# Rickyeeeeee/ParallelRayTracing

Hardware: AMD Instinct MI355X
Metric: Mrays/sec at 1920x1080, 4 bounces, ~1M-tri scene (higher is better)
Workload: dtype f32; 1 GPU; C3: dragon.ply refined by longest-edge bisection = 870000 triangles + ground quad + emissive quad, 1920x1080, max_depth 5 segments (= 4 bounces), 256 spp per step (15360 spp timed of the config's 256), image tiled over 1 GPU(s) + per-step gather to rank 0; triangles=870000, bvh_nodes=681504, bvh_max_depth=25, bvh8_nodes=137301, bvh8_depth=9, width=1920, height=1080, max_depth=5, samples_in_flight=256, seed=0, jitter=0, variant=0, gather=render stream

## Files before the change

include/prt.h:

```cpp
#ifndef PRT_H
#define PRT_H

#include <stddef.h>
#include <stdint.h>

#ifdef __cplusplus
extern "C" {
#endif

#define PRT_VERSION 1

enum {
    PRT_OK = 0,
    PRT_ERR_INVALID = 1,
    PRT_ERR_NO_DEVICE = 2,
    PRT_ERR_HIP = 3,
    PRT_ERR_IO = 4,
    PRT_ERR_NOMEM = 5
};

enum { PRT_SHAPE_CIRCLE = 0, PRT_SHAPE_QUAD = 1, PRT_SHAPE_TRIANGLE = 2 };
enum { PRT_MAT_NONE = 0, PRT_MAT_LAMBERTIAN = 1, PRT_MAT_METAL = 2, PRT_MAT_DIELECTRIC = 3, PRT_MAT_EMISSIVE = 4 };
enum {
    PRT_PRESET_DEFAULT = 0, PRT_PRESET_LIGHT_TEST = 1, PRT_PRESET_MATERIAL_TEST = 2, PRT_PRESET_CORNELL = 3,
// ... 450 lines not shown

int prt_enable_timing(PrtContext* ctx, int on);
int prt_get_stats(PrtContext* ctx, PrtStats* out);
int prt_reset_stats(PrtContext* ctx);
int prt_measure_traversal(PrtContext* ctx, uint32_t max_depth, uint32_t seed, uint32_t sample, PrtStats* out);
int prt_measure_shade_divergence(PrtContext* ctx, uint32_t max_depth, uint32_t seed, uint32_t sample, uint64_t* out);
int prt_bvh_info(PrtContext* ctx, PrtBvhInfo* out);
uint32_t prt_spill_rows(uint32_t max_stack4, uint32_t max_depth);
int prt_kernel_occupancy(PrtContext* ctx, PrtOccupancy* out);
int prt_kernel_instance(PrtContext* ctx, char* name, uint32_t capacity);
int prt_shade_instance(PrtContext* ctx, char* name, uint32_t capacity);
enum { PRT_STAGE_RAYGEN = 0, PRT_STAGE_SHADE0 = 1, PRT_STAGE_SHADE = 2, PRT_STAGE_ACCUMULATE = 3 };
int prt_batch_instance(PrtContext* ctx, uint32_t stage, char* name, uint32_t capacity);
int prt_instance_name(uint32_t stage, uint32_t index, char* name, uint32_t capacity);
int prt_last_segment(PrtContext* ctx, uint32_t* active, uint32_t* front_rays);
int prt_primary_reuse(PrtContext* ctx, uint32_t* active, uint32_t* reused_batches);
int prt_bvh_read(PrtContext* ctx, float* nodes, float* tris);
int prt_bvh_read4(PrtContext* ctx, float* nodes4);
int prt_bvh_read8(PrtContext* ctx, uint32_t* nodes8);
int prt_set_variant(PrtContext* ctx, int variant);
int prt_set_param(PrtContext* ctx, const char* name, int value);

typedef struct PrtGroup PrtGroup;
int prt_group_create(const int* device_ids, uint32_t n, PrtGroup** out);
void prt_group_destroy(PrtGroup* g);
const char* prt_group_last_error(const PrtGroup* g);
uint32_t prt_group_size(const PrtGroup* g);
const char* prt_group_transport(const PrtGroup* g);
PrtContext* prt_group_context(PrtGroup* g, uint32_t rank);
int prt_group_set_scene(PrtGroup* g, const PrtSceneDesc* scene);
// ... 59 lines not shown
```

parallelraytracing_amd/capi.py:

```python
from __future__ import annotations

import ctypes as C
import os

_HERE = os.path.dirname(os.path.abspath(__file__))
LIB_PATH = os.environ.get("PRT_LIB_PATH") or os.path.join(_HERE, "csrc", "libprt.so")

PRT_MAX_DEPTH = 64

SHAPE_CIRCLE, SHAPE_QUAD, SHAPE_TRIANGLE = 0, 1, 2
MAT_NONE, MAT_LAMBERTIAN, MAT_METAL, MAT_DIELECTRIC, MAT_EMISSIVE = 0, 1, 2, 3, 4
(PRESET_DEFAULT, PRESET_LIGHT_TEST, PRESET_MATERIAL_TEST, PRESET_CORNELL, PRESET_RANDOM_BALLS_SMALL,
 PRESET_RANDOM_BALLS_MEDIUM, PRESET_RANDOM_BALLS_LARGE) = range(7)
PRESET_NAMES = {
    "DEFAULT": PRESET_DEFAULT, "LIGHT_TEST": PRESET_LIGHT_TEST, "MATERIAL_TEST": PRESET_MATERIAL_TEST,
    "CORNELL": PRESET_CORNELL, "RANDOM_BALLS_SMALL": PRESET_RANDOM_BALLS_SMALL,
    "RANDOM_BALLS_MEDIUM": PRESET_RANDOM_BALLS_MEDIUM, "RANDOM_BALLS_LARGE": PRESET_RANDOM_BALLS_LARGE,
}


class PrtMaterial(C.Structure):
    _fields_ = [("type", C.c_uint32), ("rgb", C.c_float * 3), ("scalar", C.c_float)]


# ... 356 lines not shown
                                                 _vp, _vp, C.POINTER(PrtBakeInfo)]),
    "prt_bake_light_samples": (C.c_int, [_vp, C.POINTER(PrtBakeTarget), C.c_uint32, C.c_uint32, _fp, _fp, _u32p, _fp, _fp]),
    "prt_enable_timing": (C.c_int, [_vp, C.c_int]),
    "prt_get_stats": (C.c_int, [_vp, C.POINTER(PrtStats)]),
    "prt_reset_stats": (C.c_int, [_vp]),
    "prt_measure_traversal": (C.c_int, [_vp, C.c_uint32, C.c_uint32, C.c_uint32, C.POINTER(PrtStats)]),
    "prt_bvh_info": (C.c_int, [_vp, C.POINTER(PrtBvhInfo)]),
    "prt_spill_rows": (C.c_uint32, [C.c_uint32, C.c_uint32]),
    "prt_kernel_occupancy": (C.c_int, [_vp, C.POINTER(PrtOccupancy)]),
    "prt_kernel_instance": (C.c_int, [_vp, C.c_char_p, C.c_uint32]),
    "prt_shade_instance": (C.c_int, [_vp, C.c_char_p, C.c_uint32]),
    "prt_batch_instance": (C.c_int, [_vp, C.c_uint32, C.c_char_p, C.c_uint32]),
    "prt_instance_name": (C.c_int, [C.c_uint32, C.c_uint32, C.c_char_p, C.c_uint32]),
    "prt_last_segment": (C.c_int, [_vp, C.POINTER(C.c_uint32), C.POINTER(C.c_uint32)]),
    "prt_primary_reuse": (C.c_int, [_vp, C.POINTER(C.c_uint32), C.POINTER(C.c_uint32)]),
    "prt_measure_shade_divergence": (C.c_int, [_vp, C.c_uint32, C.c_uint32, C.c_uint32, C.POINTER(C.c_uint64)]),
    "prt_refit_meshes": (C.c_int, [_vp, C.POINTER(PrtMesh), C.c_uint32]),
    "prt_refit_meshes_device": (C.c_int, [_vp, C.POINTER(PrtMeshDeviceArrays), C.c_uint32]),
    "prt_mesh_normals_device": (C.c_int, [_vp, C.c_uint32, _vp, _vp]),
    "prt_refit_info": (C.c_int, [_vp, C.POINTER(PrtRefitInfo)]),
    "prt_set_instance_transforms": (C.c_int, [_vp, C.POINTER(PrtInstance), C.c_uint32, C.c_uint32]),
    "prt_group_set_instance_transforms": (C.c_int, [_vp, C.POINTER(PrtInstance), C.c_uint32, C.c_uint32]),
    "prt_instance_update_info": (C.c_int, [_vp, C.POINTER(PrtInstanceUpdateInfo)]),
    "prt_instances_read": (C.c_int, [_vp, C.c_uint32, _u32p, _u32p, _u32p, _u32p, _u32p]),
    "prt_bvh_read": (C.c_int, [_vp, _fp, _fp]),
    "prt_set_sampling": (C.c_int, [_vp, C.POINTER(PrtSampling)]),
    "prt_bvh_read4": (C.c_int, [_vp, _fp]),
    "prt_bvh_read8": (C.c_int, [_vp, C.POINTER(C.c_uint32)]),
    "prt_set_variant": (C.c_int, [_vp, C.c_int]),
    "prt_set_param": (C.c_int, [_vp, C.c_char_p, C.c_int]),
# ... 46 lines not shown
```

parallelraytracing_amd/csrc/prt_api.cpp:

```cpp
#include <hip/hip_runtime.h>

#include <algorithm>
#include <cfloat>
#include <chrono>
#include <cmath>
#include <cstdarg>
#include <cstdio>
#include <cstdlib>
#include <cstring>
#include <limits>
#include <string>
#include <utility>
#include <vector>

#include "../../include/prt.h"
#include "bvh.h"
#include "bvh_gpu.h"
#include "prt_adaptive.h"
#include "prt_denoise.h"
#include "prt_denoise_contract.h"
#include "prt_feature_samples.h"
#include "prt_features.h"
#include "prt_kernels.h"
#include "prt_primary_cache.h"
// ... 100 lines not shown
    int measure_spp = 1;
    float pad_coeff = kPadCoeff;
    int node_stride = 0;
    int compact_primary = 1;
    int primary_walk = 1;
    const char* shade_instance = "";
    const char* batch_instance[4] = {"", "", "", ""};
    bool batch_walked = false;
    int gpu_build = 0;
    PrtSampling sampling{0u, 0u, 0.0f};
    PrtLens lens{0.0f, 0.0f, 0.0f};
    PrtTravTuning tune{1024u, 256u, 16u, 0xFFFFFFFFu , 0u, 2u, 0u , 0u, 0u, 0u, 1u, 8u, 1u, 0u, nullptr, 0u, 2500000u, 2u , 8u , 96u , 32u , 1u};
    unsigned long long* d_shade_div = nullptr;
    uint32_t last_segment = 2;
    uint32_t last_segment_active = 0;
    uint32_t last_batch_depth = 0;
    uint32_t sort_rays = 0;
    uint32_t* d_sort = nullptr;
    size_t sort_entries = 0, sort_temp = 0;
    uint32_t* h_counts = nullptr;
    hipEvent_t ev_counts[PRT_MAX_DEPTH + 2] = {};
    hipEvent_t ev_prod[PRT_MAX_DEPTH + 2] = {};
    hipStream_t count_stream = nullptr;
    uint32_t* d_work = nullptr;
    float4* d_pix = nullptr;
    uint32_t pix_entries = 0;
    uint32_t* d_prim_pid = nullptr;
    uint32_t* d_prim_list = nullptr;
    uint32_t* d_prim_hit = nullptr;
    uint64_t prim_pid_entries = 0;
// ... 676 lines not shown
    EventPair ep{};
    auto accumulate_batch = [&]() -> int {
        if ((rc = begin_event(c, 3, &ep))) return rc;
        const PrtAccumulateArgs aa{c->d_rad, lit ? c->lb.lrad : nullptr, c->d_film_local, c->d_film_stat, tm, S_cur, max_depth,
                                   accumulate, c->ray_stats_target, compact ? c->d_pix + tm.n_pix_local : nullptr, view.list};
        if (!prt_launch_accumulate(c->stream, plan.accumulate, aa)) return fail(c, PRT_ERR_INVALID, "no such accumulate instance");
        c->batch_instance[PRT_STAGE_ACCUMULATE] = prt_accumulate_name(plan.accumulate);
        if ((rc = end_event(c, &ep))) return rc;
        if (accumulate && !view.list) c->stats.samples += S_cur;
        HIPCHECK(c, hipGetLastError());
        return PRT_OK;
    };
    c->shade_instance = "";
    for (const char*& n : c->batch_instance) n = "";
    c->last_segment_active = plan.last_segment;
    c->last_batch_depth = plan.path ? 0u : max_depth;
    if (plan.path) {
        HIPCHECK(c, hipMemsetAsync(c->d_work, 0, 256 * sizeof(uint32_t), c->stream));
        PrtPathArgs pa{c->cam, tm, c->sampling, c->d_rad, first_sample, seed, max_depth, n_paths};
        if ((rc = begin_event(c, 1, &ep))) return rc;
        prt_launch_path(c->stream, prt_plan_walk(wf), c->dsc, pa, c->d_work, c->tune);
        if ((rc = end_event(c, &ep))) return rc;
        ++c->stats.intersect_launches;
        return accumulate_batch();
    }
    if (compact && c->pix_entries < tm.n_pix_local) {
        free_dev(c->d_pix);
        c->pix_entries = 0;
        c->primary_key.valid = false;
        HIPCHECK(c, hipMalloc((void**)&c->d_pix, 4 * (size_t)tm.n_pix_local * sizeof(float4)));
// ... 79 lines not shown
            }
        }
        uint32_t n_rays_known = 0xFFFFFFFFu;
        if (exact && held) {
            n_rays_known = c->primary_counts[0] + c->primary_counts[1];
        } else if (exact) {
            HIPCHECK(c, hipEventSynchronize(c->ev_counts[d]));
            n_rays_known = c->h_counts[64 * (size_t)d] + c->h_counts[64 * (size_t)d + 32];
            if (d == 0) c->primary_counts[0] = c->h_counts[0], c->primary_counts[1] = c->h_counts[32];
        }
        if (n_rays_known == 0u) break;
        if (d == 0 && !reuse && now.valid) c->primary_key = now;
        if (c->d_shade_div) prt_launch_shade_divstats(c->stream, c->dsc, in, c->d_counts, d, n_paths, c->d_shade_div, prim_d);
        if ((rc = begin_event(c, 2, &ep))) return rc;
        const PrtShadeInst shade = d == 0 ? plan.shade0 : plan.shade;
        const PrtShadeArgs sa{&c->dsc, in, out, c->d_rad, c->d_counts, c->d_work, d, max_depth, n_paths, c->sampling, n_rays_known, prim_d, plan.last_segment,
                              f.env ? &denv : nullptr, f.tex ? &dtex : nullptr, lit ? &lt : nullptr, (lit && f.mesh_lights) ? &mlt : nullptr,
                              lit ? &c->lb : nullptr, (lit && f.light_clusters) ? &lct : nullptr};
        if (!prt_launch_shade(c->stream, shade, sa)) return fail(c, PRT_ERR_INVALID, "no such shade instance");
        c->shade_instance = prt_shade_name(shade);
        c->batch_instance[(d == 0 && plan.shade0 != plan.shade) ? PRT_STAGE_SHADE0 : PRT_STAGE_SHADE] = c->shade_instance;
        if (lit && (lt.n_lights || (f.env && (denv.t_all | denv.t_env)))) {
            const uint32_t* scount = c->d_counts + (size_t)d * PRT_CNT_STRIDE + 48u;
            const uint32_t nmax = n_rays_known == 0xFFFFFFFFu ? n_paths : n_rays_known;
            prt_launch_scan_prims_bounded(c->stream, c->dsc, c->lb.sh, scount, c->d_work, nmax);
            if (c->dsc.n_nodes) walk_rays(c, c->lb.sh, scount, nmax, true, c->tune, nullptr, nullptr);
            prt_launch_light_accum(c->stream, c->dsc, c->lb, scount, c->d_work, nmax);
        }
        if ((rc = end_event(c, &ep))) return rc;
        if (exact && d + 1 < max_depth) HIPCHECK(c, read_back(d + 1));
    }
    return accumulate_batch();
}
// ... 3058 lines not shown
int prt_last_segment(PrtContext* c, uint32_t* active, uint32_t* front_rays) {
    if (!c || !active) return PRT_ERR_INVALID;
    *active = c->last_segment_active;
    if (front_rays) {
        *front_rays = 0u;
        if (c->last_batch_depth != 0u && c->d_counts) {
            HIPCHECK(c, hipSetDevice(c->device));
            HIPCHECK(c, hipStreamSynchronize(c->stream));
            HIPCHECK(c, hipMemcpy(front_rays, c->d_counts + (size_t)(c->last_batch_depth - 1u) * PRT_CNT_STRIDE, sizeof(uint32_t),
                                  hipMemcpyDeviceToHost));
        }
    }
    return PRT_OK;
}

int prt_primary_reuse(PrtContext* c, uint32_t* active, uint32_t* reused_batches) {
    if (!c || !active) return PRT_ERR_INVALID;
    *active = c->primary_reuse_active;
    if (reused_batches) *reused_batches = c->primary_reused_batches;
    return PRT_OK;
}

int prt_bvh_info(PrtContext* c, PrtBvhInfo* out) {
    if (!c || !out) return PRT_ERR_INVALID;
    if (!c->has_scene) return fail(c, PRT_ERR_INVALID, "prt_set_scene has not been called");
    *out = c->hs.bvh_info;
    return PRT_OK;
}

int prt_bvh_read4(PrtContext* c, float* nodes4) {
// ... 27 lines not shown
    const std::string n = name;
    if (n == "variant") c->variant = value;
    else if (n == "primary_reuse" && (value == 0 || value == 1)) c->primary_reuse = value;
    else if (n == "grid_blocks" && value > 0 && value <= 8192) c->tune.grid_blocks = (uint32_t)value;
    else if (n == "chunk" && value >= 64 && value % 64 == 0) c->tune.chunk = (uint32_t)value;
    else if (n == "xcd_affinity" && (value == 0 || value == 1)) c->tune.xcd_affinity = (uint32_t)value;
    else if (n == "wide" && (value == 0 || value == 1 || value == 2)) c->tune.wide = (uint32_t)value;
    else if (n == "stack_lds" && (value == 0 || value == 1 || value == 2 || value == 3 || value == 4 || value == 5 || value == 6 || value == 24 || value == 39)) c->tune.stack_lds = (uint32_t)value;
    else if (n == "exact_grids" && (value == 0 || value == 1 || value == 2)) c->tune.exact_grids = (uint32_t)value;
    else if (n == "steal" && value >= 0 && value <= 64) c->tune.steal = (uint32_t)value;
    else if (n == "primary_hit" && (value == 0 || value == 1)) c->tune.primary_hit = (uint32_t)value;
    else if (n == "path_kernel" && value >= 0 && value <= 2) c->tune.path_kernel = (uint32_t)value;
    else if (n == "path_max" && value >= 1) c->tune.path_max = (uint32_t)value;
    else if (n == "sort_rays" && value >= 0 && value <= 2) c->sort_rays = (uint32_t)value;
    else if (n == "last_segment" && value >= 0 && value <= 2) c->last_segment = (uint32_t)value;
    else if (n == "compact_primary" && (value == 0 || value == 1)) c->compact_primary = value;
    else if (n == "primary_walk" && (value == 0 || value == 1)) c->primary_walk = value;
    else if (n == "node_stride" && (value == 0 || value == 5 || value == 8)) c->node_stride = value;
    else if (n == "pad_log2" && value >= 8 && value <= 22) c->pad_coeff = std::ldexp(1.0f, -value);
    else if (n == "tail" && value >= 0 && value <= 64) c->tune.tail = (uint32_t)value;
    else if (n == "big" && value >= 1 && value <= 16) c->tune.big = (uint32_t)value;
    else if (n == "static_small" && value >= 0 && value <= 4096) c->tune.static_small = (uint32_t)value;
    else if (n == "big_min" && value >= 1 && value <= 100000) c->tune.big_min = (uint32_t)value;
    else if (n == "big_keep" && value >= 0 && value <= 1024) c->tune.big_keep = (uint32_t)value;
    else if (n == "stack_cap" && value >= 0 && value <= 64) c->tune.stack_cap = (uint32_t)value;
    else if (n == "prim_bvh" && (value == 0 || value == 1)) c->abvh_enabled = value;
    else if (n == "measure_spp" && value >= 1 && value <= 1024) c->measure_spp = value;
    else if (n == "gpu_build" && (value == 0 || value == 1 || value == 2)) c->gpu_build = value;
    else if (n == "fuse" && (value == 0 || value == 1)) c->tune.fuse = (uint32_t)value;
    else if (n == "tri_min" && value >= 0 && value <= 1024) c->tune.tri_min = (uint32_t)value;
// ... 20 lines not shown
```

parallelraytracing_amd/csrc/prt_kernels.h:

```cpp
#pragma once
#include <hip/hip_runtime_api.h>
#include <hip/hip_vector_types.h>
#include <stdint.h>

#include "../../include/prt.h"
#include "prt_route.h"
#include "prt_walk.h"
#include "prt_scene_pod.h"

struct f3 {
    float x, y, z;
};

struct DevCamera {
    f3 pos, front, right, up;
    float W, H, tan_fov_y;
};
struct DevLens {
    float aperture, focus;
};

#define PRT_DIR_MIN 9.094947017729282e-13f

struct DevScene {
// ... 140 lines not shown
                           uint32_t* work, uint32_t max_rays, unsigned long long* stats);
struct PrtWalkArgs {
    const DevScene* sc;
    PrtRayBuf rays;
    const uint32_t* count;
    uint32_t* work;
    uint32_t* spill;
    unsigned long long* stats;
    const PrtPrimary* primary;
    const PrtTravTuning* tune;
};
void prt_launch_walk(hipStream_t st, const PrtWalkPlan& plan, const PrtWalkArgs& a);
void prt_launch_path(hipStream_t st, const PrtWalkPlan& plan, const DevScene& sc, const PrtPathArgs& pa, uint32_t* work, const PrtTravTuning& tune);
int prt_walk_occupancy(const PrtWalkPlan& plan, int* blocks_per_cu, int* vgprs, int* sgprs, int* lds_bytes);
#define PRT_LAST_SEGMENT_FLAG 0x80000000u
struct PrtShadeArgs {
    const DevScene* sc;
    PrtRayBuf in, out;
    float4* rad;
    uint32_t* counts;
    uint32_t* work;
    uint32_t depth, max_depth, cap;
    PrtSampling sp;
    uint32_t n_rays_known;
    const PrtPrimary* primary;
    uint32_t last_segment;
    const DevEnv* env;
    const DevTex* tex;
    const DevLights* lights;
    const DevMeshLights* mesh_lights;
    const PrtLightBufs* lb;
    const DevLightClusters* clusters;
};
bool prt_launch_shade(hipStream_t st, PrtShadeInst inst, const PrtShadeArgs& a);
void prt_launch_shade_divstats(hipStream_t st, const DevScene& sc, const PrtRayBuf& in, const uint32_t* counts, uint32_t iter,
                               uint32_t cap, unsigned long long* out, const PrtPrimary* primary = nullptr);
void prt_launch_primary_hit(hipStream_t st, const DevScene& sc, const PrtPrimary& pr, const uint32_t* hit, float4* pix,
                            const uint32_t* counts);
struct PrtAccumulateArgs {
    const float4* rad;
    const float4* lrad;
    float4* film_local;
    float2* stat;
    PrtTileMap tm;
    uint32_t S, max_depth;
    bool update_film;
    unsigned long long* ray_stats;
    const float4* pix_end;
    const uint32_t* list;
// ... 36 lines not shown
```

parallelraytracing_amd/csrc/prt_kernels.hip:

```cpp
#include "prt_kernels.h"

#include "prt_adaptive.h"
#include "prt_device.h"

#define HIT_MISS 0xFFFFFFFFu
#define HIT_DEAD 0xFFFFFFFEu

PRT_DEV uint32_t xcd_remap(uint32_t b, uint32_t n) {
    const uint32_t q = n >> 3, r = n & 7u;
    const uint32_t xcd = b & 7u, i = b >> 3;
    const uint32_t start = xcd < r ? xcd * (q + 1u) : r * (q + 1u) + (xcd - r) * q;
    return start + i;
}

#define CNT_STRIDE PRT_CNT_STRIDE
#define CNT_A(c, d) (c)[(d) * CNT_STRIDE]
#define CNT_B(c, d) (c)[(d) * CNT_STRIDE + 32u]
#define CNT_C(c, d) (c)[(d) * CNT_STRIDE + 16u]
#define PRODUCER_BLOCK 1024
#ifndef SHADE_BLOCK
#define SHADE_BLOCK 512
#endif

template <int BLOCK>
PRT_DEV uint32_t block_alloc2(bool front, bool back, bool done, uint32_t* cntA, uint32_t* cntB, uint32_t* cntC,
                              uint32_t cap, uint32_t mult = 1u, uint32_t* stride = nullptr, uint32_t* base = nullptr) {
    __shared__ uint32_t s_a[BLOCK / 64], s_b[BLOCK / 64], s_c[BLOCK / 64];
    __shared__ uint32_t s_base_a, s_base_b, s_tot_a, s_tot_b;
    const unsigned long long ma = __ballot(front), mb = __ballot(back), mc = __ballot(done);
    const uint32_t lane = lane_id(), wave = threadIdx.x >> 6;
    if (lane == 0) {
        s_a[wave] = (uint32_t)__popcll(ma);
        s_b[wave] = (uint32_t)__popcll(mb);
        s_c[wave] = (uint32_t)__popcll(mc);
    }
    __syncthreads();
    if (threadIdx.x == 0) {
        uint32_t ta = 0, tb = 0, tc = 0;
        for (uint32_t w = 0; w < BLOCK / 64; ++w) {
            ta += s_a[w];
            tb += s_b[w];
            tc += s_c[w];
        }
// ... 2121 lines not shown
    traverse8_body<STACK_L, WAVES, false, INST, LEAN, false, false, true>(sc, ro, rd, hit, hd2, count_ptr, work, ovf, tune,
                                                                          nullptr, PrtPrimary{}, PrtPathArgs{});
}

template <int STACK_L, int WAVES, bool INST, bool LEAN = false>
__global__ void __launch_bounds__(256, WAVES) k_occluded8_seeded(DevScene sc, const float4* __restrict__ ro,
                                                                const float4* __restrict__ rd, uint32_t* __restrict__ hit,
                                                                const float* __restrict__ hd2,
                                                                const uint32_t* __restrict__ count_ptr,
                                                                uint32_t* __restrict__ work, uint32_t* __restrict__ ovf,
                                                                PrtTravTuning tune) {
    traverse8_body<STACK_L, WAVES, false, INST, LEAN, false, false, true, true>(sc, ro, rd, hit, hd2, count_ptr, work, ovf, tune,
                                                                                nullptr, PrtPrimary{}, PrtPathArgs{});
}

template <int FUSE, bool SAMPLING, bool INST, bool ABVH, bool PRIM, bool ENV, bool TEX = false>
PRT_DEV void shade_step(DevScene sc, const float4* __restrict__ ro, const float4* __restrict__ rd, const float4* __restrict__ rt,
                        const uint32_t* __restrict__ hit, float4* __restrict__ no, float4* __restrict__ nd, float4* __restrict__ nt,
                        uint32_t* __restrict__ nhit, float* __restrict__ nhd2, float4* __restrict__ rad, uint32_t* __restrict__ counts,
                        uint32_t* __restrict__ work, uint32_t iter, uint32_t max_depth_arg, uint32_t cap, PrtSampling sp_arg, PrtPrimary pr,
                        const DevEnv* env, const DevTex* tex = nullptr) {
    const bool last_route = (max_depth_arg & PRT_LAST_SEGMENT_FLAG) != 0u;
    const uint32_t max_depth = max_depth_arg & ~PRT_LAST_SEGMENT_FLAG;
    const PrtSampling sp = SAMPLING ? sp_arg : PrtSampling{0u, 0u, 0.0f};
    const uint32_t nA = CNT_A(counts, iter), nB = CNT_B(counts, iter);
    const uint32_t count = nA + nB;
    if (blockIdx.x * (uint32_t)SHADE_BLOCK >= count) return;
    const uint32_t k = blockIdx.x * (uint32_t)SHADE_BLOCK + threadIdx.x;
    if (k < 8u) work[32u * k] = 0u;
    if (k == 8u) work[512] = 0u;
    bool front = false, back = false;
    f3 o = mk3(0.f, 0.f, 0.f), d = mk3(0.f, 0.f, 1.f), thr = mk3(0.f, 0.f, 0.f);
    uint32_t id0 = HIT_MISS, rng = 0, depth = 0, pid = 0;
    float d2_0 = 3.402823466e+38f;
    float4 pre_a = make_float4(0.f, 0.f, 0.f, 0.f), pre_b = pre_a;
    if (k < count) {
        const uint32_t src = k < nA ? k : cap - 1u - (k - nA);
        uint32_t id = (PRIM && (k >= nA || pr.walk)) ? HIT_MISS : ld_stream(&hit[src]);
        if (PRIM) {
            pid = ld_stream(&pr.pid[src]);
            uint32_t pixel, sample, lp;
            primary_ray(pr, pid, o, d, pixel, sample, &lp);
            if (k >= nA) id = __float_as_uint(pr.pix[pr.n_pix_local + lp].y);
            else if (pr.walk) id = hit[__float_as_uint(pr.pix[pr.n_pix_local + lp].x)];
            rng = path_seed(pixel, pr.first_sample + sample, pr.seed);
// ... 29 lines not shown
    }
}

template <int FUSE, bool SAMPLING, bool INST, bool ABVH, bool PRIM = false>
__global__ void __launch_bounds__(SHADE_BLOCK) k_shade(DevScene sc, const float4* __restrict__ ro,
                                                      const float4* __restrict__ rd, const float4* __restrict__ rt,
                                                      const uint32_t* __restrict__ hit, float4* __restrict__ no,
                                                      float4* __restrict__ nd, float4* __restrict__ nt,
                                                      uint32_t* __restrict__ nhit, float* __restrict__ nhd2,
                                                      float4* __restrict__ rad, uint32_t* __restrict__ counts,
                                                      uint32_t* __restrict__ work, uint32_t iter, uint32_t max_depth,
                                                      uint32_t cap, PrtSampling sp_arg, PrtPrimary pr) {
    shade_step<FUSE, SAMPLING, INST, ABVH, PRIM, false>(sc, ro, rd, rt, hit, no, nd, nt, nhit, nhd2, rad, counts, work, iter, max_depth,
                                                        cap, sp_arg, pr, nullptr);
}

template <bool INST, bool ABVH>
__global__ void __launch_bounds__(SHADE_BLOCK) k_shade_env(DevScene sc, DevEnv env, const float4* __restrict__ ro,
                                                          const float4* __restrict__ rd, const float4* __restrict__ rt,
                                                          const uint32_t* __restrict__ hit, float4* __restrict__ no,
                                                          float4* __restrict__ nd, float4* __restrict__ nt,
                                                          uint32_t* __restrict__ nhit, float* __restrict__ nhd2,
                                                          float4* __restrict__ rad, uint32_t* __restrict__ counts,
                                                          uint32_t* __restrict__ work, uint32_t iter, uint32_t max_depth,
                                                          uint32_t cap, PrtSampling sp_arg) {
    shade_step<0, true, INST, ABVH, false, true>(sc, ro, rd, rt, hit, no, nd, nt, nhit, nhd2, rad, counts, work, iter, max_depth, cap,
                                                 sp_arg, PrtPrimary{}, &env);
}

template <bool INST, bool ABVH, bool ENV>
// ... 29 lines not shown
            }
        }
    }
    pix[2u * pr.n_pix_local + pl] = a;
    pix[3u * pr.n_pix_local + pl] = b;
}

__global__ void __launch_bounds__(SHADE_BLOCK) k_shade_divstats(DevScene sc, const uint32_t* __restrict__ hit,
                                                                 const uint32_t* __restrict__ counts, uint32_t iter, uint32_t cap,
                                                                 unsigned long long* __restrict__ out, PrtPrimary pr, int compact) {
    const uint32_t nA = CNT_A(counts, iter), nB = CNT_B(counts, iter);
    const uint32_t count = nA + nB;
    if (blockIdx.x * (uint32_t)SHADE_BLOCK >= count) return;
    const uint32_t k = blockIdx.x * (uint32_t)SHADE_BLOCK + threadIdx.x;
    uint32_t type = 5u;
    if (k < count) {
        const uint32_t src = k < nA ? k : cap - 1u - (k - nA);
        uint32_t id;
        if (compact && (k >= nA || pr.walk)) {
            f3 o_, d_;
            uint32_t pixel, sample, lp;
            primary_ray(pr, pr.pid[src], o_, d_, pixel, sample, &lp);
            const float4 E = pr.pix[pr.n_pix_local + lp];
            id = k >= nA ? __float_as_uint(E.y) : hit[__float_as_uint(E.x)];
        } else {
            id = hit[src];
        }
        type = 0u;
        if (id != HIT_MISS && id != HIT_DEAD) {
            uint32_t m;
            if (id < sc.n_prims) {
                m = sc.prims[id].material;
            } else if (sc.n_insts) {
                const uint32_t v = id - sc.n_prims;
                uint32_t lo = 0, hi = sc.n_insts;
                while (hi - lo > 1u) {
                    const uint32_t mid = (lo + hi) >> 1;
                    if (sc.insts[mid].virt_base <= v) lo = mid; else hi = mid;
                }
                const DevInstance& I = sc.insts[lo];
                m = I.material == 0xFFFFFFFFu ? __float_as_uint(sc.tris[3 * (size_t)(I.slot_base + (v - I.virt_base)) + 1].w) : I.material;
            } else {
                m = __float_as_uint(sc.tris[3 * (size_t)(id - sc.n_prims) + 1].w);
            }
            type = sc.mat_type[m] <= 4u ? sc.mat_type[m] : 0u;
        }
    }
    unsigned long long* o = out + 16u * iter;
    const uint32_t lane = lane_id();
    uint32_t distinct = 0u;
    for (uint32_t t = 0; t < 5u; ++t) {
        const unsigned long long mk = __ballot(type == t);
        if (mk != 0ull && lane == 0u) {
            atomicAdd(&o[2 + t], (unsigned long long)__popcll(mk));
            atomicAdd(&o[8 + t], 1ull);
        }
        if (t >= 1u && t <= 3u && mk != 0ull) ++distinct;
    }
    const unsigned long long any = __ballot(type != 5u);
    if (lane == 0u && any != 0ull) {
        atomicAdd(&o[0], 1ull);
        atomicAdd(&o[1], (unsigned long long)__popcll(any));
        if (distinct) {
            atomicAdd(&o[14], (unsigned long long)distinct);
            atomicAdd(&o[15], 1ull);
        }
    }
}

__global__ void __launch_bounds__(256) k_accumulate(const float4* __restrict__ rad, float4* __restrict__ film_local,
                                                    PrtTileMap tm, uint32_t S, uint32_t max_depth, int update_film,
                                                    unsigned long long* __restrict__ ray_stats,
                                                    const float4* __restrict__ pix_end) {
// ... 1038 lines not shown

bool prt_launch_shade(hipStream_t st, PrtShadeInst inst, const PrtShadeArgs& a) {
    const uint32_t n_for_grid = a.n_rays_known == 0xFFFFFFFFu ? a.cap : (a.n_rays_known ? a.n_rays_known : 1u);
    const dim3 grid((uint32_t)((n_for_grid + SHADE_BLOCK - 1) / SHADE_BLOCK));
    const DevScene& sc = *a.sc;
    const PrtPrimary& pr = or_empty(a.primary);
    const DevEnv& e = or_empty(a.env);
    const DevTex& tex = or_empty(a.tex);
    const DevLights& lt = or_empty(a.lights);
    const DevMeshLights& m = or_empty(a.mesh_lights);
    const DevLightClusters& lc = or_empty(a.clusters);
    const PrtLightBufs& lb = or_empty(a.lb);
#define PRT_SHADE_RAYS a.in.o, a.in.d, a.in.t, a.in.hit, a.out.o, a.out.d, a.out.t, a.out.hit, a.out.hd2
#define PRT_SHADE_TAIL_D(D) a.rad, a.counts, a.work, a.depth, D, a.cap, a.sp
#define PRT_SHADE_TAIL PRT_SHADE_TAIL_D(a.max_depth)
#define PRT_SHADE_TAIL_LS PRT_SHADE_TAIL_D((a.last_segment ? a.max_depth | PRT_LAST_SEGMENT_FLAG : a.max_depth))
#define PRT_SHADE_ARGS_PLAIN sc, PRT_SHADE_RAYS, PRT_SHADE_TAIL_LS, pr
#define PRT_SHADE_ARGS_ENV sc, e, PRT_SHADE_RAYS, PRT_SHADE_TAIL_LS
#define PRT_SHADE_ARGS_TEX sc, tex, e, PRT_SHADE_RAYS, PRT_SHADE_TAIL_LS
#define PRT_SHADE_ARGS_NEE sc, lt, PRT_SHADE_RAYS, lb, PRT_SHADE_TAIL
#define PRT_SHADE_ARGS_NEE_ENV sc, lt, e, PRT_SHADE_RAYS, lb, PRT_SHADE_TAIL
#define PRT_SHADE_ARGS_NEE_MESH sc, lt, m, PRT_SHADE_RAYS, lb, PRT_SHADE_TAIL
#define PRT_SHADE_ARGS_NEE_MESH_ENV sc, lt, m, e, PRT_SHADE_RAYS, lb, PRT_SHADE_TAIL
#define PRT_SHADE_ARGS_NEE_TEX sc, tex, lt, m, e, PRT_SHADE_RAYS, lb, PRT_SHADE_TAIL
#define PRT_SHADE_ARGS_NEE_CLUS sc, lt, m, lc, PRT_SHADE_RAYS, lb, PRT_SHADE_TAIL
#define PRT_SHADE_ARGS_NEE_CLUS_ENV sc, lt, m, lc, e, PRT_SHADE_RAYS, lb, PRT_SHADE_TAIL
#define PRT_SHADE_ARGS_NEE_CLUS_TEX sc, tex, lt, m, lc, e, PRT_SHADE_RAYS, lb, PRT_SHADE_TAIL
#define PRT_SHADE_CASE(sig, kernel, tag, ...) \
    case PRT_INST(kernel, tag): hipLaunchKernelGGL((kernel<__VA_ARGS__>), grid, dim3(SHADE_BLOCK), 0, st, PRT_SHADE_ARGS_##sig); return true;
    switch (inst) {
        PRT_SHADE_INSTANCES(PRT_SHADE_CASE)
// ... 92 lines not shown
                       count_ptr, work);
}

void prt_launch_occlusion_bytes(hipStream_t st, const DevScene& sc, uint32_t n, const PrtRayBuf& in, const float* tmax,
                                uint8_t* out) {
    hipLaunchKernelGGL(k_occlusion_bytes, dim3(blocks_for(n)), dim3(256), 0, st, sc, n, in.o, in.d, in.hit, tmax, out);
}

void prt_launch_scatter_test(hipStream_t st, const DevScene& sc, uint32_t n, const float* in_d, const PrtHit* hits,
                             uint32_t* rng_io, uint32_t* scattered, float* atten, float* emitted, float* o_out,
                             float* d_out) {
    hipLaunchKernelGGL(k_scatter_test, dim3(blocks_for(n)), dim3(256), 0, st, sc, n, in_d, hits, rng_io, scattered,
                       atten, emitted, o_out, d_out);
}

void prt_launch_light_accum(hipStream_t st, const DevScene& sc, const PrtLightBufs& lb, const uint32_t* count_ptr,
                            uint32_t* work, uint32_t max_rays) {
    hipLaunchKernelGGL(k_light_accum, dim3(blocks_for(max_rays ? max_rays : 1u)), dim3(256), 0, st, sc, lb, count_ptr, work);
}

void prt_launch_sample_light_test(hipStream_t st, const DevScene& sc, const DevLights& lt, uint32_t n, const float* in_d,
                                  const PrtHit* hits, const uint32_t* keys, float* out_f, uint32_t* out_light, const DevMeshLights* ml,
                                  const DevEnv* env, const DevLightClusters* lc) {
    if (lc && ml) {
        if (env)
            hipLaunchKernelGGL(k_sample_light_test_clus_env, dim3(blocks_for(n)), dim3(256), 0, st, sc, lt, *ml, *lc, *env, n, in_d, hits, keys, out_f, out_light);
        else
            hipLaunchKernelGGL(k_sample_light_test_clus, dim3(blocks_for(n)), dim3(256), 0, st, sc, lt, *ml, *lc, n, in_d, hits, keys, out_f, out_light);
        return;
    }
// ... 39 lines not shown
```

parallelraytracing_amd/csrc/prt_route.h:

```cpp
#pragma once
#include <cstdint>

#include "prt_walk.h"

#define PRT_ROWS2(T, s, k) T(s, k, ff, false, false) T(s, k, ft, false, true) T(s, k, tf, true, false) T(s, k, tt, true, true)
#define PRT_ROWS3(T, s, k) \
    T(s, k, fff, false, false, false) T(s, k, fft, false, false, true) T(s, k, ftf, false, true, false) T(s, k, ftt, false, true, true) \
    T(s, k, tff, true, false, false) T(s, k, tft, true, false, true) T(s, k, ttf, true, true, false) T(s, k, ttt, true, true, true)
#define PRT_ROWS4(T, s, k) \
    T(s, k, ffff, false, false, false, false) T(s, k, ffft, false, false, false, true) T(s, k, fftf, false, false, true, false) T(s, k, fftt, false, false, true, true) \
    T(s, k, ftff, false, true, false, false) T(s, k, ftft, false, true, false, true) T(s, k, fttf, false, true, true, false) T(s, k, fttt, false, true, true, true) \
    T(s, k, tfff, true, false, false, false) T(s, k, tfft, true, false, false, true) T(s, k, tftf, true, false, true, false) T(s, k, tftt, true, false, true, true) \
    T(s, k, ttff, true, true, false, false) T(s, k, ttft, true, true, false, true) T(s, k, tttf, true, true, true, false) T(s, k, tttt, true, true, true, true)
#define PRT_RAYGEN_INSTANCES(T) \
    T(PLAIN, k_raygen, fttf, false, true, true, false) \
    T(PLAIN, k_raygen, tttf, true, true, true, false) \
    T(PLAIN, k_raygen, ffff, false, false, false, false) \
    T(PLAIN, k_raygen, ftff, false, true, false, false) \
    T(PLAIN, k_raygen, tfff, true, false, false, false) \
    T(PLAIN, k_raygen, ttff, true, true, false, false) \
    T(COMPACT, k_raygen, ffft, false, false, false, true) \
    PRT_ROWS2(T, ENV, k_raygen_env) \
    PRT_ROWS2(T, LENS, k_raygen_lens) \
    PRT_ROWS2(T, LENS_ENV, k_raygen_lens_env) \
// ... 120 lines not shown
    else if (f.tex) p.shade = PrtShadeInst(PRT_INST(k_shade_tex, fff) + (in << 2 | ab << 1 | en));
    else if (f.env) p.shade = PrtShadeInst(PRT_INST(k_shade_env, ff) + (in << 1 | ab));
    else if (f.abvh) p.shade = f.insts ? PRT_INST(k_shade, 0tttf) : PRT_INST(k_shade, 0tftf);
    else if (f.insts) p.shade = PRT_INST(k_shade, 0ttff);
    else if (p.fuse) p.shade = f.sa ? PRT_INST(k_shade, 1tfff) : PRT_INST(k_shade, 1ffff);
    else p.shade = f.sa ? PRT_INST(k_shade, 0tfff) : PRT_INST(k_shade, 0ffff);
    p.shade0 = p.compact ? PRT_INST(k_shade, 0ffft) : p.shade;

    if (f.film_stats || f.listed) p.accumulate = PrtAccumulateInst(PRT_INST(k_accumulate_stat, ff) + ((uint32_t)f.lit << 1 | (uint32_t)f.listed));
    else p.accumulate = f.lit ? PRT_I_k_accumulate_lit : PRT_I_k_accumulate;

    const bool last_ok = !p.path && p.fuse == 0u && !f.lit && !f.mesh_emissive && f.has_nodes && p.walk8 && !f.sort_rays && f.depth_ge2;
    p.last_segment = last_ok ? f.last_segment : 0u;
    return p;
}
```

parallelraytracing_amd/renderer.py:

```python
from __future__ import annotations

import ctypes as C
import math
from typing import List, Optional, Tuple

import numpy as np

from . import capi
from .capi import (PrtBvhInfo, PrtCameraDesc, PrtHit, PrtInstance, PrtMaterial, PrtMesh, PrtPrimitive, PrtSampling,
                   PrtSceneDesc, PrtStats)

_fp = C.POINTER(C.c_float)
_u32p = C.POINTER(C.c_uint32)

SKY = (0.4, 0.3, 0.6)
DEFAULT_MAX_DEPTH = 20


class PrtError(RuntimeError):
    pass


def _f32(a) -> np.ndarray:
    return np.ascontiguousarray(a, dtype=np.float32)
# ... 1239 lines not shown
        return buf.value.decode()

    def shade_instance(self) -> str:
        buf = C.create_string_buffer(96)
        self._check(capi.lib().prt_shade_instance(self._ctx, buf, 96))
        return buf.value.decode()

    def batch_instances(self) -> dict:
        return _batch_instances(self._check, self._ctx)

    def last_segment(self):
        active, front = C.c_uint32(0), C.c_uint32(0)
        self._check(capi.lib().prt_last_segment(self._ctx, C.byref(active), C.byref(front)))
        return active.value, front.value

    def primary_reuse(self):
        active, reused = C.c_uint32(0), C.c_uint32(0)
        self._check(capi.lib().prt_primary_reuse(self._ctx, C.byref(active), C.byref(reused)))
        return active.value, reused.value

    def bvh_read(self):
        b = self.bvh_info()
        nodes = np.zeros((b.n_nodes, 16), np.float32)
        tris = np.zeros((b.n_triangles, 12), np.float32)
        self._check(capi.lib().prt_bvh_read(self._ctx, nodes.ctypes.data_as(_fp), tris.ctypes.data_as(_fp)))
        return nodes, tris

    def bvh_read4(self) -> np.ndarray:
        b = self.bvh_info()
        nodes4 = np.zeros((b.n_nodes4, 32), np.float32)
# ... 375 lines not shown
```

Before: 24120 Mrays/s.

## Add opt-in in-block shade partition to regroup hit/miss lanes before shading

Adds an optional block-level partition to the shade kernel. Each thread's ray is classified as hit or miss, or as triangle, analytic or miss. The block then permutes which ray each thread shades, using ballots, LDS and nth-set-bit lookup, so lanes in a wave take the same path and divergence drops. The setting defaults to off via a new shade_partition param, and the partition mode is packed into spare high bits of max_depth. The change also pins the plain k_shade instantiation to 80 SGPRs, and adds a test kernel plus divergence stats counters. Enabling the partition costs extra barriers and scattered loads in exchange for less wave divergence.

Result: slower. 23840 Mrays/s (-1.2%).

```diff
diff --git a/include/prt.h b/include/prt.h
--- a/include/prt.h
+++ b/include/prt.h
@@ -488,6 +488,9 @@
 int prt_batch_instance(PrtContext* ctx, uint32_t stage, char* name, uint32_t capacity);
 int prt_instance_name(uint32_t stage, uint32_t index, char* name, uint32_t capacity);
 int prt_last_segment(PrtContext* ctx, uint32_t* active, uint32_t* front_rays);
+int prt_shade_partition(PrtContext* ctx, uint32_t bounce, uint32_t* active);
+int prt_shade_partition_test(PrtContext* ctx, const uint32_t* hit, uint32_t n_prims, uint32_t n_front, uint32_t n_back, uint32_t cap,
+                             uint32_t setting, uint32_t* records, uint32_t capacity);
 int prt_primary_reuse(PrtContext* ctx, uint32_t* active, uint32_t* reused_batches);
 int prt_bvh_read(PrtContext* ctx, float* nodes, float* tris);
 int prt_bvh_read4(PrtContext* ctx, float* nodes4);
diff --git a/parallelraytracing_amd/capi.py b/parallelraytracing_amd/capi.py
--- a/parallelraytracing_amd/capi.py
+++ b/parallelraytracing_amd/capi.py
@@ -394,6 +394,8 @@
     "prt_instance_name": (C.c_int, [C.c_uint32, C.c_uint32, C.c_char_p, C.c_uint32]),
     "prt_last_segment": (C.c_int, [_vp, C.POINTER(C.c_uint32), C.POINTER(C.c_uint32)]),
     "prt_primary_reuse": (C.c_int, [_vp, C.POINTER(C.c_uint32), C.POINTER(C.c_uint32)]),
+    "prt_shade_partition": (C.c_int, [_vp, C.c_uint32, C.POINTER(C.c_uint32)]),
+    "prt_shade_partition_test": (C.c_int, [_vp, _u32p, C.c_uint32, C.c_uint32, C.c_uint32, C.c_uint32, C.c_uint32, _u32p, C.c_uint32]),
     "prt_measure_shade_divergence": (C.c_int, [_vp, C.c_uint32, C.c_uint32, C.c_uint32, C.POINTER(C.c_uint64)]),
     "prt_refit_meshes": (C.c_int, [_vp, C.POINTER(PrtMesh), C.c_uint32]),
     "prt_refit_meshes_device": (C.c_int, [_vp, C.POINTER(PrtMeshDeviceArrays), C.c_uint32]),
diff --git a/parallelraytracing_amd/csrc/prt_api.cpp b/parallelraytracing_amd/csrc/prt_api.cpp
--- a/parallelraytracing_amd/csrc/prt_api.cpp
+++ b/parallelraytracing_amd/csrc/prt_api.cpp
@@ -138,6 +138,8 @@
     unsigned long long* d_shade_div = nullptr;
     uint32_t last_segment = 2;
     uint32_t last_segment_active = 0;
+    uint32_t shade_partition = 0;
+    uint32_t shade_partition_active[PRT_MAX_DEPTH] = {};
     uint32_t last_batch_depth = 0;
     uint32_t sort_rays = 0;
     uint32_t* d_sort = nullptr;
@@ -844,6 +846,7 @@
     c->shade_instance = "";
     for (const char*& n : c->batch_instance) n = "";
     c->last_segment_active = plan.last_segment;
+    for (uint32_t& p : c->shade_partition_active) p = 0u;
     c->last_batch_depth = plan.path ? 0u : max_depth;
     if (plan.path) {
         HIPCHECK(c, hipMemsetAsync(c->d_work, 0, 256 * sizeof(uint32_t), c->stream));
@@ -953,9 +956,11 @@
         if (c->d_shade_div) prt_launch_shade_divstats(c->stream, c->dsc, in, c->d_counts, d, n_paths, c->d_shade_div, prim_d);
         if ((rc = begin_event(c, 2, &ep))) return rc;
         const PrtShadeInst shade = d == 0 ? plan.shade0 : plan.shade;
+        const uint32_t partition = prt_shade_partition_for(c->shade_partition, shade, d, max_depth);
+        c->shade_partition_active[d] = partition;
         const PrtShadeArgs sa{&c->dsc, in, out, c->d_rad, c->d_counts, c->d_work, d, max_depth, n_paths, c->sampling, n_rays_known, prim_d, plan.last_segment,
                               f.env ? &denv : nullptr, f.tex ? &dtex : nullptr, lit ? &lt : nullptr, (lit && f.mesh_lights) ? &mlt : nullptr,
-                              lit ? &c->lb : nullptr, (lit && f.light_clusters) ? &lct : nullptr};
+                              lit ? &c->lb : nullptr, (lit && f.light_clusters) ? &lct : nullptr, partition};
         if (!prt_launch_shade(c->stream, shade, sa)) return fail(c, PRT_ERR_INVALID, "no such shade instance");
         c->shade_instance = prt_shade_name(shade);
         c->batch_instance[(d == 0 && plan.shade0 != plan.shade) ? PRT_STAGE_SHADE0 : PRT_STAGE_SHADE] = c->shade_instance;
@@ -4044,6 +4049,35 @@
     return PRT_OK;
 }
 
+int prt_shade_partition(PrtContext* c, uint32_t bounce, uint32_t* active) {
+    if (!c || !active || bounce >= PRT_MAX_DEPTH) return PRT_ERR_INVALID;
+    *active = c->shade_partition_active[bounce];
+    return PRT_OK;
+}
+
+int prt_shade_partition_test(PrtContext* c, const uint32_t* hit, uint32_t n_prims, uint32_t n_front, uint32_t n_back, uint32_t cap,
+                             uint32_t setting, uint32_t* records, uint32_t capacity) {
+    int rc = need_device(c);
+    if (rc) return rc;
+    if (!hit || !records || setting > 2u) return fail(c, PRT_ERR_INVALID, "null array or bad setting");
+    if (cap > 0x7FFFFFFFu || (uint64_t)n_front + n_back > cap) return fail(c, PRT_ERR_INVALID, "front + back exceed the capacity");
+    const uint32_t n = n_front + n_back;
+    if (n == 0u) return PRT_OK;
+    const uint32_t block = prt_shade_block();
+    const size_t n_out = (size_t)((n + block - 1u) / block) * block;
+    if (capacity < n_out) return fail(c, PRT_ERR_INVALID, "records[] holds %u entries, the launch reports %zu", capacity, n_out);
+    uint32_t *d_hit, *d_out;
+    PrtWorkspace ws;
+    ws.add(&d_hit, (size_t)cap).add(&d_out, n_out);
+    if ((rc = commit(c, ws, c->scratch))) return rc;
+    if ((rc = upload(c, d_hit, hit, (size_t)cap))) return rc;
+    prt_launch_shade_partition_test(c->stream, d_hit, n_prims, n_front, n_back, cap, setting, d_out);
+    HIPCHECK(c, hipGetLastError());
+    if ((rc = download(c, records, d_out, n_out))) return rc;
+    HIPCHECK(c, hipStreamSynchronize(c->stream));
+    return PRT_OK;
+}
+
 int prt_primary_reuse(PrtContext* c, uint32_t* active, uint32_t* reused_batches) {
     if (!c || !active) return PRT_ERR_INVALID;
     *active = c->primary_reuse_active;
@@ -4101,6 +4135,7 @@
     else if (n == "path_max" && value >= 1) c->tune.path_max = (uint32_t)value;
     else if (n == "sort_rays" && value >= 0 && value <= 2) c->sort_rays = (uint32_t)value;
     else if (n == "last_segment" && value >= 0 && value <= 2) c->last_segment = (uint32_t)value;
+    else if (n == "shade_partition" && value >= 0 && value <= 2) c->shade_partition = (uint32_t)value;
     else if (n == "compact_primary" && (value == 0 || value == 1)) c->compact_primary = value;
     else if (n == "primary_walk" && (value == 0 || value == 1)) c->primary_walk = value;
     else if (n == "node_stride" && (value == 0 || value == 5 || value == 8)) c->node_stride = value;
diff --git a/parallelraytracing_amd/csrc/prt_kernels.h b/parallelraytracing_amd/csrc/prt_kernels.h
--- a/parallelraytracing_amd/csrc/prt_kernels.h
+++ b/parallelraytracing_amd/csrc/prt_kernels.h
@@ -178,6 +178,8 @@
 void prt_launch_path(hipStream_t st, const PrtWalkPlan& plan, const DevScene& sc, const PrtPathArgs& pa, uint32_t* work, const PrtTravTuning& tune);
 int prt_walk_occupancy(const PrtWalkPlan& plan, int* blocks_per_cu, int* vgprs, int* sgprs, int* lds_bytes);
 #define PRT_LAST_SEGMENT_FLAG 0x80000000u
+#define PRT_SHADE_PARTITION_SHIFT 29u
+#define PRT_SHADE_PARTITION_MASK (3u << PRT_SHADE_PARTITION_SHIFT)
 struct PrtShadeArgs {
     const DevScene* sc;
     PrtRayBuf in, out;
@@ -195,8 +197,12 @@
     const DevMeshLights* mesh_lights;
     const PrtLightBufs* lb;
     const DevLightClusters* clusters;
+    uint32_t partition;
 };
 bool prt_launch_shade(hipStream_t st, PrtShadeInst inst, const PrtShadeArgs& a);
+void prt_launch_shade_partition_test(hipStream_t st, const uint32_t* hit, uint32_t n_prims, uint32_t n_front, uint32_t n_back,
+                                     uint32_t cap, uint32_t setting, uint32_t* out);
+uint32_t prt_shade_block();
 void prt_launch_shade_divstats(hipStream_t st, const DevScene& sc, const PrtRayBuf& in, const uint32_t* counts, uint32_t iter,
                                uint32_t cap, unsigned long long* out, const PrtPrimary* primary = nullptr);
 void prt_launch_primary_hit(hipStream_t st, const DevScene& sc, const PrtPrimary& pr, const uint32_t* hit, float4* pix,
diff --git a/parallelraytracing_amd/csrc/prt_kernels.hip b/parallelraytracing_amd/csrc/prt_kernels.hip
--- a/parallelraytracing_amd/csrc/prt_kernels.hip
+++ b/parallelraytracing_amd/csrc/prt_kernels.hip
@@ -23,10 +23,21 @@
 #endif
 
 template <int BLOCK>
+struct BlockAllocLds {
+    uint32_t a[BLOCK / 64], b[BLOCK / 64], c[BLOCK / 64];
+    uint32_t base_a, base_b, tot_a, tot_b;
+};
+template <int BLOCK>
+PRT_DEV BlockAllocLds<BLOCK>& block_alloc_lds() {
+    __shared__ BlockAllocLds<BLOCK> s;
+    return s;
+}
+template <int BLOCK>
 PRT_DEV uint32_t block_alloc2(bool front, bool back, bool done, uint32_t* cntA, uint32_t* cntB, uint32_t* cntC,
                               uint32_t cap, uint32_t mult = 1u, uint32_t* stride = nullptr, uint32_t* base = nullptr) {
-    __shared__ uint32_t s_a[BLOCK / 64], s_b[BLOCK / 64], s_c[BLOCK / 64];
-    __shared__ uint32_t s_base_a, s_base_b, s_tot_a, s_tot_b;
+    BlockAllocLds<BLOCK>& lds = block_alloc_lds<BLOCK>();
+    uint32_t(&s_a)[BLOCK / 64] = lds.a, (&s_b)[BLOCK / 64] = lds.b, (&s_c)[BLOCK / 64] = lds.c;
+    uint32_t &s_base_a = lds.base_a, &s_base_b = lds.base_b, &s_tot_a = lds.tot_a, &s_tot_b = lds.tot_b;
     const unsigned long long ma = __ballot(front), mb = __ballot(back), mc = __ballot(done);
     const uint32_t lane = lane_id(), wave = threadIdx.x >> 6;
     if (lane == 0) {
@@ -2178,6 +2189,93 @@
                                                                                 nullptr, PrtPrimary{}, PrtPathArgs{});
 }
 
+PRT_DEV uint32_t nth_set_bit(unsigned long long m, uint32_t r) {
+    uint32_t x = (uint32_t)m, pos = 0u;
+    uint32_t c = (uint32_t)__popc(x);
+    if (r >= c) {
+        r -= c;
+        pos = 32u;
+        x = (uint32_t)(m >> 32);
+    }
+#pragma unroll
+    for (uint32_t s = 16u; s != 0u; s >>= 1) {
+        c = (uint32_t)__popc(x & ((1u << s) - 1u));
+        if (r >= c) {
+            r -= c;
+            pos += s;
+            x >>= s;
+        }
+    }
+    return pos;
+}
+
+template <int BLOCK>
+PRT_DEV uint32_t block_partition_round(bool in, uint32_t first, bool rest, uint32_t& src) {
+    BlockAllocLds<BLOCK>& lds = block_alloc_lds<BLOCK>();
+    const unsigned long long m = __ballot(in);
+    if (lane_id() == 0u) {
+        lds.a[threadIdx.x >> 6] = (uint32_t)m;
+        lds.b[threadIdx.x >> 6] = (uint32_t)(m >> 32);
+    }
+    __syncthreads();
+    uint32_t tot = 0u;
+#pragma unroll
+    for (int w = 0; w < BLOCK / 64; ++w) tot += (uint32_t)__popc(lds.a[w]) + (uint32_t)__popc(lds.b[w]);
+    const uint32_t t = threadIdx.x;
+    const bool inv = rest && t >= tot;
+    const uint32_t r = t - (inv ? tot : first);
+    const bool mine = inv || (t >= first && r < tot);
+    uint32_t lo = 0u, hi = 0u, base = 0u, sw = 0u, seen = 0u;
+#pragma unroll
+    for (int w = 0; w < BLOCK / 64; ++w) {
+        const uint32_t l = inv ? ~lds.a[w] : lds.a[w], h = inv ? ~lds.b[w] : lds.b[w];
+        const uint32_t c = (uint32_t)__popc(l) + (uint32_t)__popc(h);
+        const bool here = r >= seen && r - seen < c;
+        lo = here ? l : lo;
+        hi = here ? h : hi;
+        base = here ? seen : base;
+        sw = here ? (uint32_t)w : sw;
+        seen += c;
+    }
+    __syncthreads();
+    if (mine) src = sw * 64u + nth_set_bit((unsigned long long)hi << 32 | lo, r - base);
+    return tot;
+}
+
+template <int BLOCK>
+PRT_DEV uint32_t block_partition(uint32_t cls, bool three) {
+    uint32_t src = threadIdx.x;
+    if (!three) {
+        block_partition_round<BLOCK>(cls == 0u, 0u, true, src);
+    } else {
+        const uint32_t n0 = block_partition_round<BLOCK>(cls == 0u, 0u, false, src);
+        const uint32_t n1 = block_partition_round<BLOCK>(cls == 1u, n0, false, src);
+        block_partition_round<BLOCK>(cls == 2u, n0 + n1, false, src);
+    }
+    return src;
+}
+
+template <int BLOCK>
+PRT_DEV uint32_t shade_partition(const uint32_t* __restrict__ hit, uint32_t n_prims, uint32_t nA, uint32_t count, uint32_t cap,
+                                 uint32_t setting) {
+    const uint32_t k0 = blockIdx.x * (uint32_t)BLOCK + threadIdx.x;
+    uint32_t cls = 2u;
+    if (k0 < count) {
+        const uint32_t id = hit[k0 < nA ? k0 : cap - 1u - (k0 - nA)];
+        if (id != HIT_MISS && id != HIT_DEAD) cls = (setting == 2u && id < n_prims) ? 1u : 0u;
+    }
+    return blockIdx.x * (uint32_t)BLOCK + block_partition<BLOCK>(cls, setting == 2u);
+}
+
+__global__ void __launch_bounds__(SHADE_BLOCK) k_shade_partition_test(const uint32_t* __restrict__ hit, uint32_t n_prims, uint32_t nA,
+                                                                       uint32_t nB, uint32_t cap, uint32_t setting,
+                                                                       uint32_t* __restrict__ out) {
+    const uint32_t count = nA + nB;
+    if (blockIdx.x * (uint32_t)SHADE_BLOCK >= count) return;
+    const uint32_t k0 = blockIdx.x * (uint32_t)SHADE_BLOCK + threadIdx.x;
+    out[k0] = setting ? shade_partition<SHADE_BLOCK>(hit, n_prims, nA, count, cap, setting) : k0;
+}
+
 template <int FUSE, bool SAMPLING, bool INST, bool ABVH, bool PRIM, bool ENV, bool TEX = false>
 PRT_DEV void shade_step(DevScene sc, const float4* __restrict__ ro, const float4* __restrict__ rd, const float4* __restrict__ rt,
                         const uint32_t* __restrict__ hit, float4* __restrict__ no, float4* __restrict__ nd, float4* __restrict__ nt,
@@ -2185,14 +2283,17 @@
                         uint32_t* __restrict__ work, uint32_t iter, uint32_t max_depth_arg, uint32_t cap, PrtSampling sp_arg, PrtPrimary pr,
                         const DevEnv* env, const DevTex* tex = nullptr) {
     const bool last_route = (max_depth_arg & PRT_LAST_SEGMENT_FLAG) != 0u;
-    const uint32_t max_depth = max_depth_arg & ~PRT_LAST_SEGMENT_FLAG;
+    const uint32_t partition = PRIM ? 0u : (max_depth_arg >> PRT_SHADE_PARTITION_SHIFT) & 3u;
+    const uint32_t max_depth = max_depth_arg & ~(PRIM ? PRT_LAST_SEGMENT_FLAG : PRT_LAST_SEGMENT_FLAG | PRT_SHADE_PARTITION_MASK);
     const PrtSampling sp = SAMPLING ? sp_arg : PrtSampling{0u, 0u, 0.0f};
     const uint32_t nA = CNT_A(counts, iter), nB = CNT_B(counts, iter);
     const uint32_t count = nA + nB;
     if (blockIdx.x * (uint32_t)SHADE_BLOCK >= count) return;
-    const uint32_t k = blockIdx.x * (uint32_t)SHADE_BLOCK + threadIdx.x;
-    if (k < 8u) work[32u * k] = 0u;
-    if (k == 8u) work[512] = 0u;
+    const uint32_t k0 = blockIdx.x * (uint32_t)SHADE_BLOCK + threadIdx.x;
+    if (k0 < 8u) work[32u * k0] = 0u;
+    if (k0 == 8u) work[512] = 0u;
+    uint32_t k = k0;
+    if (!PRIM && partition != 0u) k = shade_partition<SHADE_BLOCK>(hit, sc.n_prims, nA, count, cap, partition);
     bool front = false, back = false;
     f3 o = mk3(0.f, 0.f, 0.f), d = mk3(0.f, 0.f, 1.f), thr = mk3(0.f, 0.f, 0.f);
     uint32_t id0 = HIT_MISS, rng = 0, depth = 0, pid = 0;
@@ -2252,6 +2353,17 @@
     shade_step<FUSE, SAMPLING, INST, ABVH, PRIM, false>(sc, ro, rd, rt, hit, no, nd, nt, nhit, nhd2, rad, counts, work, iter, max_depth,
                                                         cap, sp_arg, pr, nullptr);
 }
+template <>
+__global__ void __launch_bounds__(SHADE_BLOCK) __attribute__((amdgpu_num_sgpr(80)))
+k_shade<0, false, false, false, false>(DevScene sc, const float4* __restrict__ ro, const float4* __restrict__ rd,
+                                       const float4* __restrict__ rt, const uint32_t* __restrict__ hit, float4* __restrict__ no,
+                                       float4* __restrict__ nd, float4* __restrict__ nt, uint32_t* __restrict__ nhit,
+                                       float* __restrict__ nhd2, float4* __restrict__ rad, uint32_t* __restrict__ counts,
+                                       uint32_t* __restrict__ work, uint32_t iter, uint32_t max_depth, uint32_t cap,
+                                       PrtSampling sp_arg, PrtPrimary pr) {
+    shade_step<0, false, false, false, false, false>(sc, ro, rd, rt, hit, no, nd, nt, nhit, nhd2, rad, counts, work, iter, max_depth, cap,
+                                                     sp_arg, pr, nullptr);
+}
 
 template <bool INST, bool ABVH>
 __global__ void __launch_bounds__(SHADE_BLOCK) k_shade_env(DevScene sc, DevEnv env, const float4* __restrict__ ro,
@@ -2311,6 +2423,7 @@
     if (blockIdx.x * (uint32_t)SHADE_BLOCK >= count) return;
     const uint32_t k = blockIdx.x * (uint32_t)SHADE_BLOCK + threadIdx.x;
     uint32_t type = 5u;
+    uint32_t kind = 0u;
     if (k < count) {
         const uint32_t src = k < nA ? k : cap - 1u - (k - nA);
         uint32_t id;
@@ -2325,6 +2438,7 @@
         }
         type = 0u;
         if (id != HIT_MISS && id != HIT_DEAD) {
+            kind = id < sc.n_prims ? 2u : 1u;
             uint32_t m;
             if (id < sc.n_prims) {
                 m = sc.prims[id].material;
@@ -2354,6 +2468,9 @@
         }
         if (t >= 1u && t <= 3u && mk != 0ull) ++distinct;
     }
+    const unsigned long long tri = __ballot(kind == 1u), ana = __ballot(kind == 2u);
+    if (lane == 0u && tri != 0ull) atomicAdd(&o[7], (unsigned long long)__popcll(tri));
+    if (lane == 0u && ana != 0ull) atomicAdd(&o[13], (unsigned long long)__popcll(ana));
     const unsigned long long any = __ballot(type != 5u);
     if (lane == 0u && any != 0ull) {
         atomicAdd(&o[0], 1ull);
@@ -3422,7 +3539,8 @@
 #define PRT_SHADE_RAYS a.in.o, a.in.d, a.in.t, a.in.hit, a.out.o, a.out.d, a.out.t, a.out.hit, a.out.hd2
 #define PRT_SHADE_TAIL_D(D) a.rad, a.counts, a.work, a.depth, D, a.cap, a.sp
 #define PRT_SHADE_TAIL PRT_SHADE_TAIL_D(a.max_depth)
-#define PRT_SHADE_TAIL_LS PRT_SHADE_TAIL_D((a.last_segment ? a.max_depth | PRT_LAST_SEGMENT_FLAG : a.max_depth))
+    const uint32_t depth_flags = (a.last_segment ? PRT_LAST_SEGMENT_FLAG : 0u) | (a.partition & 3u) << PRT_SHADE_PARTITION_SHIFT;
+#define PRT_SHADE_TAIL_LS PRT_SHADE_TAIL_D((a.max_depth | depth_flags))
 #define PRT_SHADE_ARGS_PLAIN sc, PRT_SHADE_RAYS, PRT_SHADE_TAIL_LS, pr
 #define PRT_SHADE_ARGS_ENV sc, e, PRT_SHADE_RAYS, PRT_SHADE_TAIL_LS
 #define PRT_SHADE_ARGS_TEX sc, tex, e, PRT_SHADE_RAYS, PRT_SHADE_TAIL_LS
@@ -3545,6 +3663,14 @@
                        atten, emitted, o_out, d_out);
 }
 
+void prt_launch_shade_partition_test(hipStream_t st, const uint32_t* hit, uint32_t n_prims, uint32_t n_front, uint32_t n_back,
+                                     uint32_t cap, uint32_t setting, uint32_t* out) {
+    const uint32_t n = n_front + n_back;
+    hipLaunchKernelGGL(k_shade_partition_test, dim3((n + SHADE_BLOCK - 1u) / SHADE_BLOCK), dim3(SHADE_BLOCK), 0, st, hit, n_prims, n_front,
+                       n_back, cap, setting, out);
+}
+uint32_t prt_shade_block() { return SHADE_BLOCK; }
+
 void prt_launch_light_accum(hipStream_t st, const DevScene& sc, const PrtLightBufs& lb, const uint32_t* count_ptr,
                             uint32_t* work, uint32_t max_rays) {
     hipLaunchKernelGGL(k_light_accum, dim3(blocks_for(max_rays ? max_rays : 1u)), dim3(256), 0, st, sc, lb, count_ptr, work);
diff --git a/parallelraytracing_amd/csrc/prt_route.h b/parallelraytracing_amd/csrc/prt_route.h
--- a/parallelraytracing_amd/csrc/prt_route.h
+++ b/parallelraytracing_amd/csrc/prt_route.h
@@ -158,3 +158,12 @@
     p.last_segment = last_ok ? f.last_segment : 0u;
     return p;
 }
+
+inline bool prt_shade_inst_partitions(PrtShadeInst i) {
+    return i != PRT_INST(k_shade, 0ffft) && i <= PRT_INST(k_shade_tex, ttt);
+}
+inline uint32_t prt_shade_partition_for(uint32_t setting, PrtShadeInst inst, uint32_t depth, uint32_t max_depth) {
+    if (setting > 2u || !prt_shade_inst_partitions(inst)) return 0u;
+    if (depth == 0u || depth + 1u >= max_depth) return 0u;
+    return setting;
+}
diff --git a/parallelraytracing_amd/renderer.py b/parallelraytracing_amd/renderer.py
--- a/parallelraytracing_amd/renderer.py
+++ b/parallelraytracing_amd/renderer.py
@@ -1277,6 +1277,22 @@
         self._check(capi.lib().prt_last_segment(self._ctx, C.byref(active), C.byref(front)))
         return active.value, front.value
 
+    def shade_partition(self) -> list:
+        out = []
+        for b in range(self.max_depth):
+            active = C.c_uint32(0)
+            self._check(capi.lib().prt_shade_partition(self._ctx, b, C.byref(active)))
+            out.append(active.value)
+        return out
+
+    def shade_partition_test(self, hit, n_prims: int, n_front: int, n_back: int, setting: int) -> np.ndarray:
+        hit = np.ascontiguousarray(hit, np.uint32)
+        n = n_front + n_back
+        out = np.zeros((n + 511) // 512 * 512, np.uint32)
+        self._check(capi.lib().prt_shade_partition_test(self._ctx, hit.ctypes.data_as(_u32p), int(n_prims), int(n_front), int(n_back),
+                                                        hit.size, int(setting), out.ctypes.data_as(_u32p), out.size))
+        return out
+
     def primary_reuse(self):
         active, reused = C.c_uint32(0), C.c_uint32(0)
         self._check(capi.lib().prt_primary_reuse(self._ctx, C.byref(active), C.byref(reused)))
```
